# nquach/TEE_optical_flow

Hardware: AMD Instinct MI355X
Metric: frame-pairs/sec @512x512 DualTVL1 (higher is better)
Workload: dtype f32

## Files before the change

tee_optical_flow_amd/csrc/teeflow.hip:

```cpp
#include "teeflow_kernels.hip.h"
#include "teeflow_deepflow.hip.h"
#include "teeflow_sor_rt.hip.h"
#include "teeflow_analysis.hip.h"
#include "teeflow_wase.hip.h"
#include "teeflow_saliency.hip.h"
#include "../../include/teeflow.h"
#include <rccl/rccl.h>
#include <dlfcn.h>

#include <chrono>
#include <cmath>
#include <cstdarg>
#include <cstdio>
#include <cstring>
#include <cstdlib>
#include <deque>
#include <string>
#include <atomic>
#include <condition_variable>
#include <functional>
#include <mutex>
#include <thread>
#include <map>
#include <vector>
// ... 239 lines not shown
        h->iters_cap >= (size_t)h->cap * (size_t)h->nlev * (size_t)h->P.warps * 2)
        return TF_OK;
    HIPC(h, hipStreamSynchronize(h->stream));
    free_buffers(h);
    h->nlev = compute_levels(h->P, H, W, h->lv);
    const size_t cap = (size_t)want_cap, fcap = 2 * cap;
    for (int l = 0; l < h->nlev; ++l) HIPC(h, hipMalloc(&h->pyr[l], fcap * h->lv[l].plane * sizeof(float)));
    if (h->P.variant == TF_VARIANT_CUDA)
        for (int l = 0; l < h->nlev; ++l) {
            HIPC(h, hipMalloc(&h->gxl[l], fcap * h->lv[l].plane * sizeof(float)));
            HIPC(h, hipMalloc(&h->gyl[l], fcap * h->lv[l].plane * sizeof(float)));
        }
    h->alloc_variant = h->P.variant;
    const size_t pl = (size_t)h->lv[0].plane * cap * sizeof(float);
    HIPC(h, hipMalloc(&h->cwx, pl)); HIPC(h, hipMalloc(&h->cwy, pl)); HIPC(h, hipMalloc(&h->crho, pl));
    for (int k = 0; k < 2; ++k) {
        HIPC(h, hipMalloc(&h->sb.u1[k], pl)); HIPC(h, hipMalloc(&h->sb.u2[k], pl));
        HIPC(h, hipMalloc(&h->sb.p11[k], pl)); HIPC(h, hipMalloc(&h->sb.p12[k], pl));
        HIPC(h, hipMalloc(&h->sb.p21[k], pl)); HIPC(h, hipMalloc(&h->sb.p22[k], pl));
    }
    HIPC(h, hipMalloc(&h->ctl, cap * sizeof(PairCtl)));
    h->errstride = total;
    HIPC(h, hipMalloc(&h->errs, cap * (size_t)h->errstride * sizeof(u64)));
    h->iters_cap = cap * (size_t)h->nlev * (size_t)h->P.warps * 2;
    HIPC(h, hipMalloc(&h->iters_dev, h->iters_cap * sizeof(int)));
    h->H = H; h->W = W; h->cap = want_cap;
    h->alloc_scale_step = h->P.scale_step; h->alloc_nscales = h->P.nscales;
    return TF_OK;
}

int ensure_staging(tf_handle* h, size_t u8_bytes, size_t flow_bytes)
{
    if (h->st_u8_bytes < u8_bytes) {
        if (h->st_u8) (void)hipFree(h->st_u8);
        h->st_u8 = nullptr; h->st_u8_bytes = 0;
        HIPC(h, hipMalloc(&h->st_u8, u8_bytes)); h->st_u8_bytes = u8_bytes;
    }
    if (h->st_flow_bytes < flow_bytes) {
        if (h->st_flow) (void)hipFree(h->st_flow);
        h->st_flow = nullptr; h->st_flow_bytes = 0;
        HIPC(h, hipMalloc(&h->st_flow, flow_bytes)); h->st_flow_bytes = flow_bytes;
    }
    return TF_OK;
}

inline dim3 grid64x4(const Geom& g, int z) { return dim3((g.w + 63) / 64, (g.h + 3) / 4, z); }

struct StageTotals {
    double iter_bytes = 0, total_bytes = 0;
};

bool rows_ok(const tf_handle* h, const Geom& g, int B)
{
    return h->iter_variant >= 1 && g.w <= h->max_strip_width && (long long)g.h * B >= h->min_rows_work;
}

bool two_per_launch(const tf_handle* h, bool cuda_variant, int inner)
{
    return cuda_variant || (h->iter_variant >= 2 && inner % 2 == 0);
}

void strip_shape(const tf_handle* h, const Geom& g, int B, int* R, int* QX, int* RY, int* threads)
{
    const int qx = (g.w + 3) / 4;
    int ry = 256 / qx;
    if (ry < 1) ry = 1;
    *QX = qx; *RY = ry;
    *threads = qx * ry <= 256 ? 256 : (qx * ry + 63) / 64 * 64;
    long long n = (long long)g.h * B / ((long long)h->strip_blocks * ry);
    if (n < 2) n = 2;
    if (n > 16) n = 16;
    *R = ry * (int)n;
}

void launch_iter2(tf_handle* h, const Iter2Args& A, int B, hipStream_t s)
{
    const Geom& g = A.a.g;
    if (!rows_ok(h, g, B)) {
        hipLaunchKernelGGL(k_iter2_tile, dim3((g.w + T2_OW - 1) / T2_OW, (g.h + T2_OH - 1) / T2_OH, B), dim3(256), 0, s, A);
        return;
    }
    int R, QX, RY, threads;
    strip_shape(h, g, B, &R, &QX, &RY, &threads);
    const int LW = QX * 4 + 4;
    const size_t shmem = (size_t)(32 + 8 * RY * LW + 2 * (RY + 1) * LW + 2 * RY * QX) * sizeof(float);
    if (B <= 1024) {
        auto f = h->slots_cache.find(shmem * 1024 + (size_t)threads / 64);
        if (f == h->slots_cache.end()) {
            int per_cu = 0;
            (void)hipOccupancyMaxActiveBlocksPerMultiprocessor(&per_cu, k_iter2_rows, threads, shmem);
            if (per_cu < 1) per_cu = 1;
            f = h->slots_cache.emplace(shmem * 1024 + (size_t)threads / 64, per_cu * h->num_cus).first;
        }
        int slots = f->second;
        if (h->slots_pct > 0 && h->slots_pct < 100) slots = slots * h->slots_pct / 100;
        int items = 1;
        for (int n = 1; n <= B; ++n) {
            int r, sn;
            strip_rule(n, g.h, RY, slots, &r, &sn);
            if (n * sn > items) items = n * sn;
        }
        hipLaunchKernelGGL(k_iter2_rows, dim3(items, 1, 1), dim3(threads), shmem, s, A, 0, QX, RY, slots);
        return;
    }
    hipLaunchKernelGGL(k_iter2_rows, dim3((g.h + R - 1) / R, 1, B), dim3(threads), shmem, s, A, R, QX, RY, 0);
}

void launch_iter(tf_handle* h, const IterArgs& ia, int B, hipStream_t s)
{
    const Geom& g = ia.g;
    if (rows_ok(h, g, B)) {
        int R, QX, RY, threads;
        strip_shape(h, g, B, &R, &QX, &RY, &threads);
        const int LW = QX * 4 + 4;
        const size_t shmem = (size_t)(32 + 8 * RY * LW + 2 * RY * QX) * sizeof(float);
        hipLaunchKernelGGL(k_iter_rows, dim3((g.h + R - 1) / R, 1, B), dim3(threads), shmem, s, ia, R, QX, RY);
    } else {
        const dim3 gi((g.w + IT_OW - 1) / IT_OW, (g.h + IT_OH - 1) / IT_OH, B);
        hipLaunchKernelGGL(k_iter, gi, dim3(256), 0, s, ia);
    }
}

inline int warp_margin_class(int m) { return m <= 0 ? 0 : (m <= 4 ? 4 : (m <= 8 ? 8 : 16)); }
void launch_warp(tf_handle* h, const WarpArgs& wa, int B, hipStream_t s, const float* gx = nullptr, const float* gy = nullptr)
{
    const Geom& g = wa.g;
    if (h->P.variant == TF_VARIANT_CUDA) {
        WarpCudaArgs ca; ca.w = wa; ca.gx = gx; ca.gy = gy;
        hipLaunchKernelGGL(k_warp_cuda, dim3((g.w + 63) / 64, (g.h + 3) / 4, B), dim3(256), 0, s, ca);
        return;
    }
    const int M = warp_margin_class(h->warp_margin);
    const dim3 grid((g.w + WL_TW - 1) / WL_TW, (g.h + WL_TH - 1) / WL_TH, B);
    const size_t shm = (size_t)(128 + (WL_TW + 2 * (M + 4)) * (WL_TH + 2 * M + 7)) * sizeof(float);
    switch (M) {
        case 4: hipLaunchKernelGGL(k_warp_lds<4>, grid, dim3(256), shm, s, wa); break;
        case 8: hipLaunchKernelGGL(k_warp_lds<8>, grid, dim3(256), shm, s, wa); break;
        case 16: hipLaunchKernelGGL(k_warp_lds<16>, grid, dim3(256), shm, s, wa); break;
        default: hipLaunchKernelGGL(k_warp, dim3((g.w + 63) / 64, (g.h + 3) / 4, B), dim3(256), 0, s, wa); break;
    }
}

template <class Launch>
int profiled(tf_handle* h, hipStream_t s, int level, int warp, int it, Launch&& launch)
{
    if (!h->profile) { launch(); return TF_OK; }
    if (h->prof_used == h->prof_pool.size()) {
        ProfEv pe;
        hipError_t e = hipEventCreate(&pe.a);
        if (e == hipSuccess && (e = hipEventCreate(&pe.b)) != hipSuccess) (void)hipEventDestroy(pe.a);
        if (e != hipSuccess) { (void)hipGetLastError(); return fail(h, TF_ERR_HIP, "hipEventCreate failed: %s", hipGetErrorString(e)); }
        h->prof_pool.push_back(pe);
    }
    ProfEv& pe = h->prof_pool[h->prof_used++];
    pe.level = level; pe.warp = warp; pe.it = it;
    HIPC(h, hipEventRecord(pe.a, s));
    launch();
    HIPC(h, hipEventRecord(pe.b, s));
    return TF_OK;
}

int read_reports(tf_handle* h, hipStream_t s, unsigned q, unsigned* checked, bool* stop)
{
    while (*checked <= q) {
        int v = h->slots_host[*checked % SLOT_RING];
        if (v < 0) {
            if (q - *checked < (unsigned)DEFAULT_LAG) break;
            const double t0 = now_ms();
// ... 2037 lines not shown
```

tee_optical_flow_amd/csrc/teeflow_kernels.hip.h:

```cpp
#pragma once
#include <hip/hip_runtime.h>
#include <stdint.h>
#include <float.h>

#define TF_HD __host__ __device__
#include "median_net.h"

typedef unsigned long long u64;

struct Geom {
    int w, h, pitch;
    long long plane;
    long long splane;
};

struct PairCtl {
    int ubase;
    int pbase;
};

struct StateBufs {
    float* u1[2]; float* u2[2];
    float* p11[2]; float* p12[2]; float* p21[2]; float* p22[2];
};
// ... 942 lines not shown
    if (tid == 0) {
        u64 tot = 0;
        for (int w = 0; w < (int)(blockDim.x >> 6); ++w) tot += sred[w];
        atomicAdd(&errb[a.it], tot);
    }
}

#define M_EXIT 0
#define M_NORMAL 1
#define M_REPLAY 2

__device__ __forceinline__ int pair_mode2(const u64* e, int it, int total, double thr)
{
    const bool a1 = it >= 1 ? (double)e[it - 1] > thr : true;
    const bool a2 = it >= 2 ? (double)e[it - 2] > thr : true;
    if (it < total && (it == 0 || (a2 && a1))) return M_NORMAL;
    if (it >= 2 && !a2) {
        const int j = it - 2;
        const bool act = j == 0 || ((double)e[j - 2] > thr && (double)e[j - 1] > thr);
        if (act) return M_REPLAY;
    }
    return M_EXIT;
}

__device__ __forceinline__ int pair_mode_cuda(const u64* e, int it, int total, double thr, int* n_it)
{
    double prev = 0.0;
    for (int n = 0; n < it; ++n) {
        const bool calc = thr > 0.0 && (n & 1) && prev < thr;
        if (calc) {
            const double err = (double)e[n] * 0x1p-30;
            prev = err;
            if (!(err > thr)) { if (n_it) *n_it = n + 1; return M_EXIT; }
        } else prev -= thr;
    }
    if (n_it) *n_it = total;
    return it < total ? M_NORMAL : M_EXIT;
}

__device__ __forceinline__ int pair_mode(const u64* e, int it, int total, double thr_q, int variant, double thr_d)
{
    return variant ? pair_mode_cuda(e, it, total, thr_d, nullptr) : pair_mode2(e, it, total, thr_q);
}

TF_HD inline void strip_rule_min(int n, int H, int minrows, int slots, int* R, int* S)
{
    if (n < 1) n = 1;
    if (minrows < 1) minrows = 1;
    const int k = (n + slots - 1) / slots;
    int s = (int)(((long long)k * slots) / n);
    const int smax = H / minrows > 0 ? H / minrows : 1;
    if (s > smax) s = smax;
    if (s < 1) s = 1;
    int r = (H + s - 1) / s;
    *R = r;
    *S = (H + r - 1) / r;
}
TF_HD inline void strip_rule(int n, int H, int RY, int slots, int* R, int* S)
{
    strip_rule_min(n, H, 4 * RY, slots, R, S);
}

struct Iter2Args {
    IterArgs a;
    int utog_prev, ptog_prev, pzero_prev;
    int total;
};

__device__ __forceinline__ void publish_active_count2(const Iter2Args& A)
{
    const IterArgs& a = A.a;
    if (a.host_slot && blockIdx.x == 0 && blockIdx.y == 0 && blockIdx.z == 0 && threadIdx.x < 64) {
        int c = 0;
        for (int b2 = threadIdx.x; b2 < a.B; b2 += 64)
            c += pair_mode(a.err + (size_t)b2 * a.errstride, a.it, A.total, a.thr_q, a.variant, a.thr_d) != M_EXIT ? 1 : 0;
#pragma unroll
        for (int off = 32; off > 0; off >>= 1) c += __shfl_down(c, off, 64);
        if (threadIdx.x == 0) __hip_atomic_store(a.host_slot, c, __ATOMIC_RELAXED, __HIP_MEMORY_SCOPE_SYSTEM);
    }
}


struct Iter2Blk {
    int b, strip, R, QX, RY;
    bool replay, pzero;
    int uc, pc;
    int it;
    u64* errb;
    int W, H, pitch;
    long long splane;
};

__device__ __forceinline__ void iter2_rows_body(const IterArgs& a, const Iter2Blk& k, float* smem);

__global__ __launch_bounds__(512) void k_iter2_rows(Iter2Args A, int R, int QX, int RY, int slots)
{
    extern __shared__ __attribute__((aligned(16))) float smem[];
    const IterArgs& a = A.a;
    u64* sred = reinterpret_cast<u64*>(smem);

    publish_active_count2(A);
    int b = blockIdx.z, strip = blockIdx.x;
    if (slots > 0) {
        const int nchunk = (a.B + 63) >> 6, nw = (int)(blockDim.x >> 6), wv = (int)(threadIdx.x >> 6), ln = (int)(threadIdx.x & 63);
        for (int c = wv; c < nchunk; c += nw) {
            const int pb = c * 64 + ln;
            const bool on = pb < a.B && pair_mode(a.err + (size_t)pb * a.errstride, a.it, A.total, a.thr_q, a.variant, a.thr_d) != M_EXIT;
            const u64 m = __ballot(on);
            if (ln == 0) sred[c] = m;
        }
        __syncthreads();
        int nact = 0;
        for (int c = 0; c < nchunk; ++c) nact += __popcll(sred[c]);
        int S;
        strip_rule(nact, a.g.h, RY, slots, &R, &S);
        const int item = blockIdx.x;
        if (item >= nact * S) return;
        int k = item / S;
        strip = item - k * S;
        int c = 0;
        u64 m = sred[0];
        while (k >= __popcll(m)) { k -= __popcll(m); m = sred[++c]; }
        for (; k > 0; --k) m &= m - 1;
        b = c * 64 + (__ffsll((long long)m) - 1);
        __syncthreads();
    }
    u64* errb = a.err + (size_t)b * a.errstride;
    const int mode = pair_mode(errb, a.it, A.total, a.thr_q, a.variant, a.thr_d);
    if (mode == M_EXIT) return;
    const bool replay = mode == M_REPLAY;
    const PairCtl c = a.ctl[b];
    const int utog = replay ? A.utog_prev : a.utog, ptog = replay ? A.ptog_prev : a.ptog;
    Iter2Blk blk;
    blk.b = b; blk.strip = strip; blk.R = R; blk.QX = QX; blk.RY = RY; blk.replay = replay;
    blk.pzero = (replay ? A.pzero_prev : a.pzero) != 0;
    blk.uc = (c.ubase ^ utog) & 1; blk.pc = (c.pbase ^ ptog) & 1;
    blk.it = a.it; blk.errb = errb;
    blk.W = a.g.w; blk.H = a.g.h; blk.pitch = a.g.pitch; blk.splane = a.g.splane;
    iter2_rows_body(a, blk, smem);
}

__device__ __forceinline__ void iter2_rows_body(const IterArgs& a, const Iter2Blk& k, float* smem)
{
    const int b = k.b, strip = k.strip, R = k.R, QX = k.QX, RY = k.RY, uc = k.uc, pc = k.pc;
    const bool replay = k.replay, pzero = k.pzero;
    u64* errb = k.errb;
    const int LW = QX * 4 + 4;
    u64* sred = reinterpret_cast<u64*>(smem);
    float* U1a = smem + 32;
    float* U1b = U1a + 2 * RY * LW;
    float* U2a = U1b + 2 * RY * LW;
    float* U2b = U2a + 2 * RY * LW;
    float* B12 = U2b + 2 * RY * LW;
    float* B22 = B12 + (RY + 1) * LW;
    float* B11w = B22 + (RY + 1) * LW;
    float* B21w = B11w + RY * QX;
    const int tid = threadIdx.x;
    const int ty = tid / QX, tx = tid - ty * QX;
    const bool lane_on = ty < RY;
    const int W = k.W, H = k.H, pitch = k.pitch;
    const int x = tx * 4;
    const int y0 = strip * R;
    const int ngroups = (R + 3 + RY - 1) / RY;
    const size_t po = (size_t)b * (size_t)k.splane;
    const int RB = RY + 1;

    const float* __restrict__ gu1 = a.sb.u1[uc] + po;
    const float* __restrict__ gu2 = a.sb.u2[uc] + po;
    const float* __restrict__ g11 = a.sb.p11[pc] + po;
    const float* __restrict__ g12 = a.sb.p12[pc] + po;
    const float* __restrict__ g21 = a.sb.p21[pc] + po;
    const float* __restrict__ g22 = a.sb.p22[pc] + po;
    const float* __restrict__ gwx = a.wx + po;
    const float* __restrict__ gwy = a.wy + po;
    const float* __restrict__ grh = a.rho + po;
    float* __restrict__ ou1 = a.sb.u1[uc ^ 1] + po;
    float* __restrict__ ou2 = a.sb.u2[uc ^ 1] + po;
    float* __restrict__ o11 = a.sb.p11[pc ^ 1] + po;
    float* __restrict__ o12 = a.sb.p12[pc ^ 1] + po;
    float* __restrict__ o21 = a.sb.p21[pc ^ 1] + po;
    float* __restrict__ o22 = a.sb.p22[pc ^ 1] + po;

    const int yu1_lo = y0 - 1, yu1_hi = y0 + R + 1, yp1_hi = y0 + R, yout_hi = y0 + R - 1;

    float s1_u1[4], s1_u2[4], s1_wx[4], s1_wy[4], s1_r[4], s1_11[4], s1_12[4], s1_21[4], s1_22[4];
    float s2_u1[4], s2_u2[4], s2_11[4], s2_12[4], s2_21[4], s2_22[4];
#pragma unroll
    for (int i = 0; i < 4; ++i) {
        s1_u1[i] = s1_u2[i] = s1_wx[i] = s1_wy[i] = s1_r[i] = s1_11[i] = s1_12[i] = s1_21[i] = s1_22[i] = 0.f;
        s2_u1[i] = s2_u2[i] = s2_11[i] = s2_12[i] = s2_21[i] = s2_22[i] = 0.f;
    }
    bool s1_valid = false, s2_valid = false;
    unsigned inw[5];
#pragma unroll
    for (int j = 0; j < 5; ++j) inw[j] = opaque_u(x + j < W ? ~0u : 0u);
    int ring = ty + 1;
    u64 qA = 0, qB = 0;
    double accA = 0.0, accB = 0.0;

    for (int s = 0; s < ngroups + 2; ++s) {
        const int r1 = s * RY + ty;
        const int y = y0 - 1 + r1;
        const bool v1 = lane_on && s < ngroups && y >= 0 && y < H && y >= yu1_lo && y <= yu1_hi;
        const size_t row = (size_t)y * pitch + x;
        float4 u1q, u2q, wxq, wyq, rq, a11, a12, a21, a22;
        u1q = u2q = wxq = wyq = rq = a11 = a12 = a21 = a22 = make_float4(0, 0, 0, 0);
        if (v1) {
            u1q = ld4(gu1 + row); u2q = ld4(gu2 + row);
            wxq = ld4(gwx + row); wyq = ld4(gwy + row); rq = ld4(grh + row);
            if (!pzero) { a11 = ld4(g11 + row); a12 = ld4(g12 + row); a21 = ld4(g21 + row); a22 = ld4(g22 + row); }
        }
        float n_u1[4] = {0, 0, 0, 0}, n_u2[4] = {0, 0, 0, 0};
        float c11[4], c12[4], c21[4], c22[4], wxv[4], wyv[4], rv[4];
        UNPACK4(c11, a11) UNPACK4(c12, a12) UNPACK4(c21, a21) UNPACK4(c22, a22) UNPACK4(wxv, wxq) UNPACK4(wyv, wyq) UNPACK4(rv, rq)
        if (v1) {
            float4 up12 = make_float4(0, 0, 0, 0), up22 = up12;
            if (y > 0 && !pzero) { up12 = ld4(g12 + row - pitch); up22 = ld4(g22 + row - pitch); }
            float l11 = 0.f, l21 = 0.f;
            if (tx > 0 && !pzero) { l11 = g11[row - 1]; l21 = g21[row - 1]; }
            QuadU qu;
            UNPACK4(qu.u1k, u1q) UNPACK4(qu.u2k, u2q) UNPACK4(qu.wx, wxq) UNPACK4(qu.wy, wyq) UNPACK4(qu.r, rq)
            UNPACK4(qu.p11, a11) UNPACK4(qu.p12, a12) UNPACK4(qu.p21, a21) UNPACK4(qu.p22, a22)
            UNPACK4(qu.p12u, up12) UNPACK4(qu.p22u, up22)
            qu.l11 = l11; qu.l21 = l21;
            const bool isout = y >= y0 && y <= yout_hi;
            tv_u_quad_pk(a.l_t, a.theta, qu, y == 0, x == 0, n_u1, n_u2);
            const unsigned mrow = opaque_u(!replay && isout ? ~0u : 0u);
            const unsigned keep[4] = {inw[0] & mrow, inw[1] & mrow, inw[2] & mrow, inw[3] & mrow};
            accA += tv_err_quad_pk(n_u1, qu.u1k, n_u2, qu.u2k, keep);
            st4(U1a + ((s & 1) * RY + ty) * LW + x, PACK4(n_u1));
            st4(U1b + ((s & 1) * RY + ty) * LW + x, PACK4(n_u2));
        }
        __syncthreads();
        const int yb = y - RY;
        const bool v2 = s1_valid && yb <= yp1_hi;
        float p1_11[4] = {0, 0, 0, 0}, p1_12[4] = {0, 0, 0, 0}, p1_21[4] = {0, 0, 0, 0}, p1_22[4] = {0, 0, 0, 0};
        if (v2) {
            const int bp = (s - 1) & 1;
            const bool lastrow = yb >= H - 1;
            float4 dn1 = make_float4(0, 0, 0, 0), dn2 = dn1;
            if (!lastrow) {
                const float* d1 = ty < RY - 1 ? U1a + (bp * RY + ty + 1) * LW + x : U1a + ((s & 1) * RY) * LW + x;
                const float* d2 = ty < RY - 1 ? U1b + (bp * RY + ty + 1) * LW + x : U1b + ((s & 1) * RY) * LW + x;
                dn1 = ld4(d1); dn2 = ld4(d2);
            }
            float rr1 = 0.f, rr2 = 0.f;
            if (x + 4 < W) { rr1 = U1a[(bp * RY + ty) * LW + x + 4]; rr2 = U1b[(bp * RY + ty) * LW + x + 4]; }
            const unsigned mnl = opaque_u(lastrow ? 0u : ~0u);
            float dv1[4], dv2[4], u1x[4], u1y[4], u2x[4], u2y[4];
            UNPACK4(dv1, dn1) UNPACK4(dv2, dn2)
            {
                const float4 o1 = ld4(U1a + (bp * RY + ty) * LW + x), o2 = ld4(U1b + (bp * RY + ty) * LW + x);
                UNPACK4(s1_u1, o1) UNPACK4(s1_u2, o2)
            }
#pragma unroll
            for (int i = 0; i < 4; ++i) {
                const float e1 = i < 3 ? s1_u1[i + 1] : rr1, e2 = i < 3 ? s1_u2[i + 1] : rr2;
                u1x[i] = mask_f(e1 - s1_u1[i], inw[i + 1]);
                u2x[i] = mask_f(e2 - s1_u2[i], inw[i + 1]);
                u1y[i] = mask_f(dv1[i] - s1_u1[i], mnl);
                u2y[i] = mask_f(dv2[i] - s1_u2[i], mnl);
            }
            tv_p_quad_pk(a.taut, u1x, u1y, u2x, u2y, s1_11, s1_12, s1_21, s1_22, p1_11, p1_12, p1_21, p1_22);
            if (replay) {
                if (yb >= y0 && yb <= yout_hi) {
                    const size_t prow = (size_t)yb * pitch + x;
                    st4(ou1 + prow, PACK4(s1_u1)); st4(ou2 + prow, PACK4(s1_u2));
                    st4(o11 + prow, PACK4(p1_11)); st4(o12 + prow, PACK4(p1_12));
                    st4(o21 + prow, PACK4(p1_21)); st4(o22 + prow, PACK4(p1_22));
                }
            } else {
                st4(B12 + ring * LW + x, PACK4(p1_12));
                st4(B22 + ring * LW + x, PACK4(p1_22));
                B11w[ty * QX + tx] = p1_11[3];
                B21w[ty * QX + tx] = p1_21[3];
            }
        }
        bool v2u = false;
        float m_u1[4] = {0, 0, 0, 0}, m_u2[4] = {0, 0, 0, 0};
        if (!replay) {
            __syncthreads();
            v2u = v2 && yb >= y0;
            if (v2u) {
                float4 up12 = make_float4(0, 0, 0, 0), up22 = up12;
                if (yb > 0) {
                    const int ri = ring > 0 ? ring - 1 : RB - 1;
                    up12 = ld4(B12 + ri * LW + x); up22 = ld4(B22 + ri * LW + x);
                }
                float l11 = 0.f, l21 = 0.f;
                if (tx > 0) { l11 = B11w[ty * QX + tx - 1]; l21 = B21w[ty * QX + tx - 1]; }
                QuadU qu;
#pragma unroll
                for (int i = 0; i < 4; ++i) {
                    qu.u1k[i] = s1_u1[i]; qu.u2k[i] = s1_u2[i]; qu.wx[i] = s1_wx[i]; qu.wy[i] = s1_wy[i]; qu.r[i] = s1_r[i];
                    qu.p11[i] = p1_11[i]; qu.p12[i] = p1_12[i]; qu.p21[i] = p1_21[i]; qu.p22[i] = p1_22[i];
                }
                UNPACK4(qu.p12u, up12) UNPACK4(qu.p22u, up22)
                qu.l11 = l11; qu.l21 = l21;
                const bool isout = yb <= yout_hi;
                tv_u_quad_pk(a.l_t, a.theta, qu, yb == 0, x == 0, m_u1, m_u2);
                const unsigned mrow = opaque_u(isout ? ~0u : 0u);
                const unsigned keep[4] = {inw[0] & mrow, inw[1] & mrow, inw[2] & mrow, inw[3] & mrow};
                accB += tv_err_quad_pk(m_u1, s1_u1, m_u2, s1_u2, keep);
                st4(U2a + (((s - 1) & 1) * RY + ty) * LW + x, PACK4(m_u1));
                st4(U2b + (((s - 1) & 1) * RY + ty) * LW + x, PACK4(m_u2));
            }
            __syncthreads();
            const int yc = y - 2 * RY;
            if (s2_valid && yc <= yout_hi) {
                const int bq = s & 1;
                const bool lastrow = yc >= H - 1;
                float4 dn1 = make_float4(0, 0, 0, 0), dn2 = dn1;
                if (!lastrow) {
                    const float* d1 = ty < RY - 1 ? U2a + (bq * RY + ty + 1) * LW + x : U2a + ((bq ^ 1) * RY) * LW + x;
                    const float* d2 = ty < RY - 1 ? U2b + (bq * RY + ty + 1) * LW + x : U2b + ((bq ^ 1) * RY) * LW + x;
                    dn1 = ld4(d1); dn2 = ld4(d2);
                }
                float rr1 = 0.f, rr2 = 0.f;
                if (x + 4 < W) { rr1 = U2a[(bq * RY + ty) * LW + x + 4]; rr2 = U2b[(bq * RY + ty) * LW + x + 4]; }
                const unsigned mnl = opaque_u(lastrow ? 0u : ~0u);
                float dv1[4], dv2[4], r11[4], r12[4], r21[4], r22[4], u1x[4], u1y[4], u2x[4], u2y[4];
                UNPACK4(dv1, dn1) UNPACK4(dv2, dn2)
                {
                    const float4 o1 = ld4(U2a + (bq * RY + ty) * LW + x), o2 = ld4(U2b + (bq * RY + ty) * LW + x);
                    UNPACK4(s2_u1, o1) UNPACK4(s2_u2, o2)
                }
#pragma unroll
                for (int i = 0; i < 4; ++i) {
                    const float e1 = i < 3 ? s2_u1[i + 1] : rr1, e2 = i < 3 ? s2_u2[i + 1] : rr2;
                    u1x[i] = mask_f(e1 - s2_u1[i], inw[i + 1]);
                    u2x[i] = mask_f(e2 - s2_u2[i], inw[i + 1]);
                    u1y[i] = mask_f(dv1[i] - s2_u1[i], mnl);
                    u2y[i] = mask_f(dv2[i] - s2_u2[i], mnl);
                }
                tv_p_quad_pk(a.taut, u1x, u1y, u2x, u2y, s2_11, s2_12, s2_21, s2_22, r11, r12, r21, r22);
                const size_t prow = (size_t)yc * pitch + x;
                st4(ou1 + prow, PACK4(s2_u1)); st4(ou2 + prow, PACK4(s2_u2));
                st4(o11 + prow, PACK4(r11)); st4(o12 + prow, PACK4(r12));
                st4(o21 + prow, PACK4(r21)); st4(o22 + prow, PACK4(r22));
            }
        }
        else __syncthreads();
        s2_valid = v2u;
#pragma unroll
        for (int i = 0; i < 4; ++i) {
            s2_11[i] = p1_11[i]; s2_12[i] = p1_12[i]; s2_21[i] = p1_21[i]; s2_22[i] = p1_22[i];
            s1_wx[i] = wxv[i]; s1_wy[i] = wyv[i]; s1_r[i] = rv[i];
            s1_11[i] = c11[i]; s1_12[i] = c12[i]; s1_21[i] = c21[i]; s1_22[i] = c22[i];
        }
        s1_valid = v1;
        ring += RY; ring = ring >= RB ? ring - RB : ring;
        if ((s & 255) == 255) { qA += (u64)accA; qB += (u64)accB; accA = accB = 0.0; }
    }
    if (!replay) {
        qA += (u64)accA; qB += (u64)accB;
#pragma unroll
        for (int off = 32; off > 0; off >>= 1) { qA += __shfl_down(qA, off, 64); qB += __shfl_down(qB, off, 64); }
        __syncthreads();
        if ((tid & 63) == 0) { sred[tid >> 6] = qA; sred[8 + (tid >> 6)] = qB; }
        __syncthreads();
        if (tid == 0) {
            u64 ta = 0, tb = 0;
            for (int w = 0; w < (int)(blockDim.x >> 6); ++w) { ta += sred[w]; tb += sred[8 + w]; }
            atomicAdd(&errb[k.it], ta);
            atomicAdd(&errb[k.it + 1], tb);
        }
    }
}

#define T2_OW 52
#define T2_OH 13

__global__ __launch_bounds__(256) void k_iter2_tile(Iter2Args A)
{
    constexpr int LW = 68;
    __shared__ __attribute__((aligned(16))) float sA[16][LW], sB[16][LW];
    __shared__ __attribute__((aligned(16))) float s12[16][LW], s22[16][LW];
    __shared__ float s11w[16][16], s21w[16][16];
    __shared__ u64 sred[8];
    const IterArgs& a = A.a;
    publish_active_count2(A);
    const int b = blockIdx.z;
    u64* errb = a.err + (size_t)b * a.errstride;
    const int mode = pair_mode(errb, a.it, A.total, a.thr_q, a.variant, a.thr_d);
    if (mode == M_EXIT) return;
    const bool replay = mode == M_REPLAY;
    const PairCtl c = a.ctl[b];
    const int utog = replay ? A.utog_prev : a.utog, ptog = replay ? A.ptog_prev : a.ptog;
    const bool pzero = (replay ? A.pzero_prev : a.pzero) != 0;
    const int uc = (c.ubase ^ utog) & 1, pc = (c.pbase ^ ptog) & 1;
    const int tx = threadIdx.x & 15, ty = threadIdx.x >> 4;
    const int W = a.g.w, H = a.g.h, pitch = a.g.pitch;
    const int x = (int)blockIdx.x * T2_OW - 4 + tx * 4, y = (int)blockIdx.y * T2_OH - 1 + ty;
    const bool inr = x >= 0 && x < W && y >= 0 && y < H;
    const bool outq = inr && tx >= 1 && tx <= 13 && ty >= 1 && ty <= 13;
    const size_t po = (size_t)b * a.g.splane;
    const size_t row = po + (size_t)(inr ? y : 0) * pitch + (inr ? x : 0);

    unsigned inw[5];
#pragma unroll
    for (int j = 0; j < 5; ++j) inw[j] = opaque_u(x + j < W ? ~0u : 0u);
    const unsigned mnl = opaque_u(y >= H - 1 ? 0u : ~0u);
    const unsigned mout = opaque_u(outq ? ~0u : 0u);
    const unsigned keep[4] = {inw[0] & mout, inw[1] & mout, inw[2] & mout, inw[3] & mout};

    float u0_1[4], u0_2[4], wx[4], wy[4], rc[4], p0_11[4], p0_12[4], p0_21[4], p0_22[4];
    float u1_1[4], u1_2[4];
    double accA = 0.0, accB = 0.0;
    if (inr) {
        const float4 u1q = ld4(a.sb.u1[uc] + row), u2q = ld4(a.sb.u2[uc] + row);
        const float4 wxq = ld4(a.wx + row), wyq = ld4(a.wy + row), rq = ld4(a.rho + row);
        float4 a11 = make_float4(0, 0, 0, 0), a12 = a11, a21 = a11, a22 = a11, up12 = a11, up22 = a11;
        float l11 = 0.f, l21 = 0.f;
        if (!pzero) {
            a11 = ld4(a.sb.p11[pc] + row); a12 = ld4(a.sb.p12[pc] + row);
            a21 = ld4(a.sb.p21[pc] + row); a22 = ld4(a.sb.p22[pc] + row);
            if (y > 0) { up12 = ld4(a.sb.p12[pc] + row - pitch); up22 = ld4(a.sb.p22[pc] + row - pitch); }
            if (x > 0) { l11 = a.sb.p11[pc][row - 1]; l21 = a.sb.p21[pc][row - 1]; }
        }
        QuadU qu;
        UNPACK4(qu.u1k, u1q) UNPACK4(qu.u2k, u2q) UNPACK4(qu.wx, wxq) UNPACK4(qu.wy, wyq) UNPACK4(qu.r, rq)
        UNPACK4(qu.p11, a11) UNPACK4(qu.p12, a12) UNPACK4(qu.p21, a21) UNPACK4(qu.p22, a22)
        UNPACK4(qu.p12u, up12) UNPACK4(qu.p22u, up22)
        qu.l11 = l11; qu.l21 = l21;
        UNPACK4(u0_1, u1q) UNPACK4(u0_2, u2q) UNPACK4(wx, wxq) UNPACK4(wy, wyq) UNPACK4(rc, rq)
        UNPACK4(p0_11, a11) UNPACK4(p0_12, a12) UNPACK4(p0_21, a21) UNPACK4(p0_22, a22)
        tv_u_quad_pk(a.l_t, a.theta, qu, y == 0, x == 0, u1_1, u1_2);
        if (!replay) accA += tv_err_quad_pk(u1_1, u0_1, u1_2, u0_2, keep);
        st4(&sA[ty][tx * 4], PACK4(u1_1));
        st4(&sB[ty][tx * 4], PACK4(u1_2));
    }
    __syncthreads();
    float p1_11[4], p1_12[4], p1_21[4], p1_22[4];
    const bool vP1 = inr && tx <= 14 && ty <= 14;
// ... 197 lines not shown
```

Before: 2818.

## Linearize strip-kernel thread mapping into flat ring buffer over quads

Replaces the row-group (ty,tx) thread mapping in the fused two-iteration strip kernel with a flat linear walk, where each step covers T consecutive quads of the strip and neighbours are found through a 2T-entry ring buffer in LDS. This keeps every thread busy even when QX does not divide the block size, where before the lanes with ty >= RY sat idle. Column-boundary masks now come from a per-step bitmask instead of per-thread precomputed masks, and LDS sizing now depends only on thread count. It adds modular index arithmetic and carries the position state across pipeline stages, at the cost of extra register pressure and a more intricate halo correctness argument.

```diff
diff --git a/tee_optical_flow_amd/csrc/teeflow.hip b/tee_optical_flow_amd/csrc/teeflow.hip
--- a/tee_optical_flow_amd/csrc/teeflow.hip
+++ b/tee_optical_flow_amd/csrc/teeflow.hip
@@ -345,8 +345,7 @@
     }
     int R, QX, RY, threads;
     strip_shape(h, g, B, &R, &QX, &RY, &threads);
-    const int LW = QX * 4 + 4;
-    const size_t shmem = (size_t)(32 + 8 * RY * LW + 2 * (RY + 1) * LW + 2 * RY * QX) * sizeof(float);
+    const size_t shmem = (size_t)iter2_rows_lds_floats(threads) * sizeof(float);
     if (B <= 1024) {
         auto f = h->slots_cache.find(shmem * 1024 + (size_t)threads / 64);
         if (f == h->slots_cache.end()) {
diff --git a/tee_optical_flow_amd/csrc/teeflow_kernels.hip.h b/tee_optical_flow_amd/csrc/teeflow_kernels.hip.h
--- a/tee_optical_flow_amd/csrc/teeflow_kernels.hip.h
+++ b/tee_optical_flow_amd/csrc/teeflow_kernels.hip.h
@@ -1048,7 +1048,7 @@
 
 
 struct Iter2Blk {
-    int b, strip, R, QX, RY;
+    int b, strip, R, QX;
     bool replay, pzero;
     int uc, pc;
     int it;
@@ -1098,7 +1098,7 @@
     const PairCtl c = a.ctl[b];
     const int utog = replay ? A.utog_prev : a.utog, ptog = replay ? A.ptog_prev : a.ptog;
     Iter2Blk blk;
-    blk.b = b; blk.strip = strip; blk.R = R; blk.QX = QX; blk.RY = RY; blk.replay = replay;
+    blk.b = b; blk.strip = strip; blk.R = R; blk.QX = QX; blk.replay = replay;
     blk.pzero = (replay ? A.pzero_prev : a.pzero) != 0;
     blk.uc = (c.ubase ^ utog) & 1; blk.pc = (c.pbase ^ ptog) & 1;
     blk.it = a.it; blk.errb = errb;
@@ -1106,30 +1106,35 @@
     iter2_rows_body(a, blk, smem);
 }
 
+TF_HD inline int iter2_rows_lds_floats(int T)
+{
+    return 32 + 6 * 2 * T * 4 + 2 * 2 * T;
+}
+
+__device__ __forceinline__ int ring_wrap(int i, int n) { return (int)min((unsigned)i, (unsigned)(i - n)); }
+__device__ __forceinline__ unsigned bit_mask(unsigned m, int j) { return opaque_u((unsigned)((int)(m << (31 - j)) >> 31)); }
+
 __device__ __forceinline__ void iter2_rows_body(const IterArgs& a, const Iter2Blk& k, float* smem)
 {
-    const int b = k.b, strip = k.strip, R = k.R, QX = k.QX, RY = k.RY, uc = k.uc, pc = k.pc;
+    const int b = k.b, strip = k.strip, R = k.R, QX = k.QX, uc = k.uc, pc = k.pc;
     const bool replay = k.replay, pzero = k.pzero;
     u64* errb = k.errb;
-    const int LW = QX * 4 + 4;
+    const int T = (int)blockDim.x, T2 = 2 * T;
     u64* sred = reinterpret_cast<u64*>(smem);
     float* U1a = smem + 32;
-    float* U1b = U1a + 2 * RY * LW;
-    float* U2a = U1b + 2 * RY * LW;
-    float* U2b = U2a + 2 * RY * LW;
-    float* B12 = U2b + 2 * RY * LW;
-    float* B22 = B12 + (RY + 1) * LW;
-    float* B11w = B22 + (RY + 1) * LW;
-    float* B21w = B11w + RY * QX;
+    float* U1b = U1a + 4 * T2;
+    float* U2a = U1b + 4 * T2;
+    float* U2b = U2a + 4 * T2;
+    float* B12 = U2b + 4 * T2;
+    float* B22 = B12 + 4 * T2;
+    float* B11w = B22 + 4 * T2;
+    float* B21w = B11w + T2;
     const int tid = threadIdx.x;
-    const int ty = tid / QX, tx = tid - ty * QX;
-    const bool lane_on = ty < RY;
     const int W = k.W, H = k.H, pitch = k.pitch;
-    const int x = tx * 4;
     const int y0 = strip * R;
-    const int ngroups = (R + 3 + RY - 1) / RY;
+    const int nsteps = ((R + 3) * QX + T - 1) / T;
+    const int dr = T / QX, dq = T - dr * QX;
     const size_t po = (size_t)b * (size_t)k.splane;
-    const int RB = RY + 1;
 
     const float* __restrict__ gu1 = a.sb.u1[uc] + po;
     const float* __restrict__ gu2 = a.sb.u2[uc] + po;
@@ -1147,7 +1152,7 @@
     float* __restrict__ o21 = a.sb.p21[pc ^ 1] + po;
     float* __restrict__ o22 = a.sb.p22[pc ^ 1] + po;
 
-    const int yu1_lo = y0 - 1, yu1_hi = y0 + R + 1, yp1_hi = y0 + R, yout_hi = y0 + R - 1;
+    const int yp1_hi = y0 + R, yout_hi = y0 + R - 1;
 
     float s1_u1[4], s1_u2[4], s1_wx[4], s1_wy[4], s1_r[4], s1_11[4], s1_12[4], s1_21[4], s1_22[4];
     float s2_u1[4], s2_u2[4], s2_11[4], s2_12[4], s2_21[4], s2_22[4];
@@ -1157,17 +1162,19 @@
         s2_u1[i] = s2_u2[i] = s2_11[i] = s2_12[i] = s2_21[i] = s2_22[i] = 0.f;
     }
     bool s1_valid = false, s2_valid = false;
-    unsigned inw[5];
-#pragma unroll
-    for (int j = 0; j < 5; ++j) inw[j] = opaque_u(x + j < W ? ~0u : 0u);
-    int ring = ty + 1;
+    int r1 = tid / QX, c1 = tid - (tid / QX) * QX;
+    int yb = 0, xb = 0, yc = 0, xc = 0;
+    const unsigned cb_last = (1u << (W - 4 * (QX - 1))) - 1u;
+    unsigned cbb = 0, cbc = 0;
     u64 qA = 0, qB = 0;
     double accA = 0.0, accB = 0.0;
 
-    for (int s = 0; s < ngroups + 2; ++s) {
-        const int r1 = s * RY + ty;
-        const int y = y0 - 1 + r1;
-        const bool v1 = lane_on && s < ngroups && y >= 0 && y < H && y >= yu1_lo && y <= yu1_hi;
+    for (int s = 0; s < nsteps + 2; ++s) {
+        const int y = y0 - 1 + r1, x = c1 * 4;
+        const bool v1 = r1 < R + 3 && y >= 0 && y < H;
+        const int o1 = (s & 1) * T + tid;
+        const int ob = ring_wrap(o1 + T, T2);
+        const unsigned cb = c1 == QX - 1 ? cb_last : 31u;
         const size_t row = (size_t)y * pitch + x;
         float4 u1q, u2q, wxq, wyq, rq, a11, a12, a21, a22;
         u1q = u2q = wxq = wyq = rq = a11 = a12 = a21 = a22 = make_float4(0, 0, 0, 0);
@@ -1183,7 +1190,7 @@
             float4 up12 = make_float4(0, 0, 0, 0), up22 = up12;
             if (y > 0 && !pzero) { up12 = ld4(g12 + row - pitch); up22 = ld4(g22 + row - pitch); }
             float l11 = 0.f, l21 = 0.f;
-            if (tx > 0 && !pzero) { l11 = g11[row - 1]; l21 = g21[row - 1]; }
+            if (x > 0 && !pzero) { l11 = g11[row - 1]; l21 = g21[row - 1]; }
             QuadU qu;
             UNPACK4(qu.u1k, u1q) UNPACK4(qu.u2k, u2q) UNPACK4(qu.wx, wxq) UNPACK4(qu.wy, wyq) UNPACK4(qu.r, rq)
             UNPACK4(qu.p11, a11) UNPACK4(qu.p12, a12) UNPACK4(qu.p21, a21) UNPACK4(qu.p22, a22)
@@ -1191,55 +1198,56 @@
             qu.l11 = l11; qu.l21 = l21;
             const bool isout = y >= y0 && y <= yout_hi;
             tv_u_quad_pk(a.l_t, a.theta, qu, y == 0, x == 0, n_u1, n_u2);
-            const unsigned mrow = opaque_u(!replay && isout ? ~0u : 0u);
-            const unsigned keep[4] = {inw[0] & mrow, inw[1] & mrow, inw[2] & mrow, inw[3] & mrow};
+            const unsigned kb = !replay && isout ? cb : 0u;
+            const unsigned keep[4] = {bit_mask(kb, 0), bit_mask(kb, 1), bit_mask(kb, 2), bit_mask(kb, 3)};
             accA += tv_err_quad_pk(n_u1, qu.u1k, n_u2, qu.u2k, keep);
-            st4(U1a + ((s & 1) * RY + ty) * LW + x, PACK4(n_u1));
-            st4(U1b + ((s & 1) * RY + ty) * LW + x, PACK4(n_u2));
+            st4(U1a + o1 * 4, PACK4(n_u1));
+            st4(U1b + o1 * 4, PACK4(n_u2));
         }
         __syncthreads();
-        const int yb = y - RY;
         const bool v2 = s1_valid && yb <= yp1_hi;
         float p1_11[4] = {0, 0, 0, 0}, p1_12[4] = {0, 0, 0, 0}, p1_21[4] = {0, 0, 0, 0}, p1_22[4] = {0, 0, 0, 0};
         if (v2) {
-            const int bp = (s - 1) & 1;
             const bool lastrow = yb >= H - 1;
             float4 dn1 = make_float4(0, 0, 0, 0), dn2 = dn1;
             if (!lastrow) {
-                const float* d1 = ty < RY - 1 ? U1a + (bp * RY + ty + 1) * LW + x : U1a + ((s & 1) * RY) * LW + x;
-                const float* d2 = ty < RY - 1 ? U1b + (bp * RY + ty + 1) * LW + x : U1b + ((s & 1) * RY) * LW + x;
-                dn1 = ld4(d1); dn2 = ld4(d2);
+                const int d = ring_wrap(ob + QX, T2);
+                dn1 = ld4(U1a + d * 4); dn2 = ld4(U1b + d * 4);
             }
             float rr1 = 0.f, rr2 = 0.f;
-            if (x + 4 < W) { rr1 = U1a[(bp * RY + ty) * LW + x + 4]; rr2 = U1b[(bp * RY + ty) * LW + x + 4]; }
+            if (cbb & 16u) {
+                const int e = ring_wrap(ob + 1, T2);
+                rr1 = U1a[e * 4]; rr2 = U1b[e * 4];
+            }
             const unsigned mnl = opaque_u(lastrow ? 0u : ~0u);
+            const unsigned mcol[4] = {bit_mask(cbb, 1), bit_mask(cbb, 2), bit_mask(cbb, 3), bit_mask(cbb, 4)};
             float dv1[4], dv2[4], u1x[4], u1y[4], u2x[4], u2y[4];
             UNPACK4(dv1, dn1) UNPACK4(dv2, dn2)
             {
-                const float4 o1 = ld4(U1a + (bp * RY + ty) * LW + x), o2 = ld4(U1b + (bp * RY + ty) * LW + x);
-                UNPACK4(s1_u1, o1) UNPACK4(s1_u2, o2)
+                const float4 w1 = ld4(U1a + ob * 4), w2 = ld4(U1b + ob * 4);
+                UNPACK4(s1_u1, w1) UNPACK4(s1_u2, w2)
             }
 #pragma unroll
             for (int i = 0; i < 4; ++i) {
                 const float e1 = i < 3 ? s1_u1[i + 1] : rr1, e2 = i < 3 ? s1_u2[i + 1] : rr2;
-                u1x[i] = mask_f(e1 - s1_u1[i], inw[i + 1]);
-                u2x[i] = mask_f(e2 - s1_u2[i], inw[i + 1]);
+                u1x[i] = mask_f(e1 - s1_u1[i], mcol[i]);
+                u2x[i] = mask_f(e2 - s1_u2[i], mcol[i]);
                 u1y[i] = mask_f(dv1[i] - s1_u1[i], mnl);
                 u2y[i] = mask_f(dv2[i] - s1_u2[i], mnl);
             }
             tv_p_quad_pk(a.taut, u1x, u1y, u2x, u2y, s1_11, s1_12, s1_21, s1_22, p1_11, p1_12, p1_21, p1_22);
             if (replay) {
                 if (yb >= y0 && yb <= yout_hi) {
-                    const size_t prow = (size_t)yb * pitch + x;
+                    const size_t prow = (size_t)yb * pitch + xb;
                     st4(ou1 + prow, PACK4(s1_u1)); st4(ou2 + prow, PACK4(s1_u2));
                     st4(o11 + prow, PACK4(p1_11)); st4(o12 + prow, PACK4(p1_12));
                     st4(o21 + prow, PACK4(p1_21)); st4(o22 + prow, PACK4(p1_22));
                 }
             } else {
-                st4(B12 + ring * LW + x, PACK4(p1_12));
-                st4(B22 + ring * LW + x, PACK4(p1_22));
-                B11w[ty * QX + tx] = p1_11[3];
-                B21w[ty * QX + tx] = p1_21[3];
+                st4(B12 + ob * 4, PACK4(p1_12));
+                st4(B22 + ob * 4, PACK4(p1_22));
+                B11w[ob] = p1_11[3];
+                B21w[ob] = p1_21[3];
             }
         }
         bool v2u = false;
@@ -1250,11 +1258,14 @@
             if (v2u) {
                 float4 up12 = make_float4(0, 0, 0, 0), up22 = up12;
                 if (yb > 0) {
-                    const int ri = ring > 0 ? ring - 1 : RB - 1;
-                    up12 = ld4(B12 + ri * LW + x); up22 = ld4(B22 + ri * LW + x);
+                    const int ua = ring_wrap(ob + (T2 - QX), T2);
+                    up12 = ld4(B12 + ua * 4); up22 = ld4(B22 + ua * 4);
                 }
                 float l11 = 0.f, l21 = 0.f;
-                if (tx > 0) { l11 = B11w[ty * QX + tx - 1]; l21 = B21w[ty * QX + tx - 1]; }
+                if (xb > 0) {
+                    const int lf = ring_wrap(ob + (T2 - 1), T2);
+                    l11 = B11w[lf]; l21 = B21w[lf];
+                }
                 QuadU qu;
 #pragma unroll
                 for (int i = 0; i < 4; ++i) {
@@ -1264,43 +1275,44 @@
                 UNPACK4(qu.p12u, up12) UNPACK4(qu.p22u, up22)
                 qu.l11 = l11; qu.l21 = l21;
                 const bool isout = yb <= yout_hi;
-                tv_u_quad_pk(a.l_t, a.theta, qu, yb == 0, x == 0, m_u1, m_u2);
-                const unsigned mrow = opaque_u(isout ? ~0u : 0u);
-                const unsigned keep[4] = {inw[0] & mrow, inw[1] & mrow, inw[2] & mrow, inw[3] & mrow};
+                tv_u_quad_pk(a.l_t, a.theta, qu, yb == 0, xb == 0, m_u1, m_u2);
+                const unsigned kb = isout ? cbb : 0u;
+                const unsigned keep[4] = {bit_mask(kb, 0), bit_mask(kb, 1), bit_mask(kb, 2), bit_mask(kb, 3)};
                 accB += tv_err_quad_pk(m_u1, s1_u1, m_u2, s1_u2, keep);
-                st4(U2a + (((s - 1) & 1) * RY + ty) * LW + x, PACK4(m_u1));
-                st4(U2b + (((s - 1) & 1) * RY + ty) * LW + x, PACK4(m_u2));
+                st4(U2a + ob * 4, PACK4(m_u1));
+                st4(U2b + ob * 4, PACK4(m_u2));
             }
             __syncthreads();
-            const int yc = y - 2 * RY;
             if (s2_valid && yc <= yout_hi) {
-                const int bq = s & 1;
                 const bool lastrow = yc >= H - 1;
                 float4 dn1 = make_float4(0, 0, 0, 0), dn2 = dn1;
                 if (!lastrow) {
-                    const float* d1 = ty < RY - 1 ? U2a + (bq * RY + ty + 1) * LW + x : U2a + ((bq ^ 1) * RY) * LW + x;
-                    const float* d2 = ty < RY - 1 ? U2b + (bq * RY + ty + 1) * LW + x : U2b + ((bq ^ 1) * RY) * LW + x;
-                    dn1 = ld4(d1); dn2 = ld4(d2);
+                    const int d = ring_wrap(o1 + QX, T2);
+                    dn1 = ld4(U2a + d * 4); dn2 = ld4(U2b + d * 4);
                 }
                 float rr1 = 0.f, rr2 = 0.f;
-                if (x + 4 < W) { rr1 = U2a[(bq * RY + ty) * LW + x + 4]; rr2 = U2b[(bq * RY + ty) * LW + x + 4]; }
+                if (cbc & 16u) {
+                    const int e = ring_wrap(o1 + 1, T2);
+                    rr1 = U2a[e * 4]; rr2 = U2b[e * 4];
+                }
                 const unsigned mnl = opaque_u(lastrow ? 0u : ~0u);
+                const unsigned mcol[4] = {bit_mask(cbc, 1), bit_mask(cbc, 2), bit_mask(cbc, 3), bit_mask(cbc, 4)};
                 float dv1[4], dv2[4], r11[4], r12[4], r21[4], r22[4], u1x[4], u1y[4], u2x[4], u2y[4];
                 UNPACK4(dv1, dn1) UNPACK4(dv2, dn2)
                 {
-                    const float4 o1 = ld4(U2a + (bq * RY + ty) * LW + x), o2 = ld4(U2b + (bq * RY + ty) * LW + x);
-                    UNPACK4(s2_u1, o1) UNPACK4(s2_u2, o2)
+                    const float4 w1 = ld4(U2a + o1 * 4), w2 = ld4(U2b + o1 * 4);
+                    UNPACK4(s2_u1, w1) UNPACK4(s2_u2, w2)
                 }
 #pragma unroll
                 for (int i = 0; i < 4; ++i) {
                     const float e1 = i < 3 ? s2_u1[i + 1] : rr1, e2 = i < 3 ? s2_u2[i + 1] : rr2;
-                    u1x[i] = mask_f(e1 - s2_u1[i], inw[i + 1]);
-                    u2x[i] = mask_f(e2 - s2_u2[i], inw[i + 1]);
+                    u1x[i] = mask_f(e1 - s2_u1[i], mcol[i]);
+                    u2x[i] = mask_f(e2 - s2_u2[i], mcol[i]);
                     u1y[i] = mask_f(dv1[i] - s2_u1[i], mnl);
                     u2y[i] = mask_f(dv2[i] - s2_u2[i], mnl);
                 }
                 tv_p_quad_pk(a.taut, u1x, u1y, u2x, u2y, s2_11, s2_12, s2_21, s2_22, r11, r12, r21, r22);
-                const size_t prow = (size_t)yc * pitch + x;
+                const size_t prow = (size_t)yc * pitch + xc;
                 st4(ou1 + prow, PACK4(s2_u1)); st4(ou2 + prow, PACK4(s2_u2));
                 st4(o11 + prow, PACK4(r11)); st4(o12 + prow, PACK4(r12));
                 st4(o21 + prow, PACK4(r21)); st4(o22 + prow, PACK4(r22));
@@ -1315,7 +1327,9 @@
             s1_11[i] = c11[i]; s1_12[i] = c12[i]; s1_21[i] = c21[i]; s1_22[i] = c22[i];
         }
         s1_valid = v1;
-        ring += RY; ring = ring >= RB ? ring - RB : ring;
+        yc = yb; xc = xb; cbc = cbb; yb = y; xb = x; cbb = cb;
+        c1 += dq; r1 += dr;
+        if (c1 >= QX) { c1 -= QX; ++r1; }
         if ((s & 255) == 255) { qA += (u64)accA; qB += (u64)accB; accA = accB = 0.0; }
     }
     if (!replay) {
```

After: 2821 (median of 6 runs). About the same (+0.1%).
